# segments-ai/latent-diffusion-segmentation

Measured on AMD Instinct MI355X. Metric: denoising-steps/sec, higher is better.
Workload: dtype bf16; 1 GPU; 512x512 COCO-shaped latents (64x64x4), batch 8 per GPU, DDIM, self-conditioned 12-ch UNet without cross-attention (BASELINE configs[1]); batch_per_gpu=8, global_batch=8, latent=64, parallelism=dp1, ranks=1, backend=none, visible_devices=1

## Files before the change

include/ldmseg_hip_ops.h:

```cpp
#ifndef LDMSEG_HIP_OPS_H_
#define LDMSEG_HIP_OPS_H_
#include <stdint.h>
#ifdef __cplusplus
extern "C" {
#endif

int ldmseg_op_conv2d(const float* x, const float* x2, const float* w, const float* bias, int B, int Ci, int Ci2, int H,
                     int W, int Co, int k, int stride, int up, int dtype, float* out, void* stream);
int ldmseg_op_linear(const float* x, const float* w, const float* bias, const float* resid, const float* rowbias,
                     int rows_per_image, int M, int K, int N, int geglu, int silu, int splits, int dtype, float* out,
                     void* stream);
int ldmseg_op_chained_ff_out(const float* g, const float* h, const float* x, const float* w2, const float* b2, const float* wp,
                             const float* bp, int M, int C, int rows_per_image, int dtype, float* out, void* stream);
int ldmseg_op_groupnorm(const float* x, const float* x2, const float* gamma, const float* beta, int B, int C, int C2,
                        int HW, float eps, int silu, int dtype, float* out, void* stream);
int ldmseg_op_layernorm(const float* x, const float* gamma, const float* beta, int M, int C, float eps, int silu,
                        int dtype, float* out, void* stream);
int ldmseg_op_attention(const float* qkv, int B, int N, int C, int heads, int dtype, float* out, void* stream);
int ldmseg_op_attention_causal(const float* qkv, int B, int N, int C, int heads, int dtype, float* out, void* stream);
int ldmseg_op_attention_cross(const float* q, const float* kv, int B, int N, int S, int C, int heads, int dtype, float* out,
                              void* stream);
int ldmseg_op_attention_fp8(const float* qkv, int B, int N, int C, int heads, float* out, int time_iters, float* us_per_launch,
                            void* stream);
int ldmseg_op_convt2(const float* x, const float* w, const float* bias, int B, int Ci, int H, int W, int Co, int dtype,
// ... 41 lines not shown
                             const float* w2, const float* b2, const float* wp, const float* bp, int M, int C, float eps, int dtype,
                             int mode, float* out, int time_iters, float* us_per_call, void* stream);
int ldmseg_op_conv_out_tail(const float* x, const float* w, const float* bias, int B, int H, int W, float* eps_out, int ddim, int last,
                            const float* coef4, int pred_type, int clip, float clip_range, float* latents, float* cond,
                            const float* rgb, const uint8_t* known, const float* z0, const float* noise, float sa, float sb,
                            float* xin_out, void* stream);
int ldmseg_bench_igemm(const float* x, const float* x2, const float* w, const float* bias, const float* resid,
                       const float* rowbias, int B, int Ci, int Ci2, int H, int W, int Co, int k, int stride, int up, int geglu,
                       int silu, int splits, int dtype, int iters, float* us_per_launch, void* stream);
int ldmseg_bench_groupnorm(const float* gamma, const float* beta, int B, int C, int C2, int HW, int silu, int dtype, int iters,
                           float* us_per_launch, void* stream);
int ldmseg_bench_attention(const float* qkv, int B, int N, int C, int heads, int dtype, int iters, float* us_per_launch,
                           void* stream);
int ldmseg_igemm_last_kernel(char* buf, int n);
int ldmseg_op_igemm_plan(const int* desc, int dtype, int cus, char* buf, int n);
int ldmseg_op_groupnorm_plan(int B, int C, int C2, int HW, int groups, int dtype, int cus, int region_ok, char* buf, int n);
int ldmseg_op_conv_groupnorm_plan(int B, int Co, int HW, int dtype, char* buf, int n);
int ldmseg_op_attention_plan(int kind, int B, int N, int S, int C, int heads, int dtype, char* buf, int n);
int ldmseg_igemm_log(int enable);
int ldmseg_igemm_log_read(char* buf, int n);

int ldmseg_op_fastdiv(const int* n, int count, int d, int* q, void* stream);

#ifdef __cplusplus
}
#endif
#endif
```

latent-diffusion-segmentation_amd/csrc/engine.hip:

```cpp
#include <hip/hip_runtime.h>

#include <algorithm>
#include <array>
#include <cmath>
#include <cstdio>
#include <cstring>
#include <string>
#include <unordered_map>
#include <vector>

#include "../../include/ldmseg_hip.h"
#include "attn_plan.h"
#include "kernels.h"

using namespace ldmseg;

namespace {

thread_local std::string g_err;
int g_plan_epoch = 0;
int g_gnfold_mode = 1;
int g_ffp_mode = 1;
int fail(int code, const std::string& msg) {
  g_err = msg;
// ... 2423 lines not shown
  if (key == 8) { groupnorm_set_variant(value); ++g_plan_epoch; return 0; }
  if (key == 9) { igemm_set_cm_mode(value); ++g_plan_epoch; return 0; }
  if (key == 10) { groupnorm_set_coop(value, groupnorm_knob(11)); return 0; }
  if (key == 11) { groupnorm_set_coop(groupnorm_knob(10), value); return 0; }
  if (key == 12) { mlp_fused_set_mode(value); ++g_plan_epoch; return 0; }
  if (key == 13) { mlp_fused_set_dbg(value); return 0; }
  if (key == 14) { step_tail_set_mode(value); ++g_plan_epoch; return 0; }
  if (key == 16) { proj_qkv_set_mode(value); ++g_plan_epoch; return 0; }
  if (key == 15) { attention_mx_set_mode(value); ++g_plan_epoch; return 0; }
  if (key == 23) { igemm_set_cf_mode(value); ++g_plan_epoch; return 0; }
  if (key == 24) { igemm_set_table_override(value); ++g_plan_epoch; return 0; }
  if (key == 19) { igemm_set_xt_mode(value); ++g_plan_epoch; return 0; }
  if (key == 20) { g_ffp_mode = value ? 1 : 0; ++g_plan_epoch; return 0; }
  if (key == 22) { g_gnfold_mode = value < 0 ? 0 : value; ++g_plan_epoch; return 0; }
  if (key == 21) { igemm_set_up4_mode(value); ++g_plan_epoch; return 0; }
  if (key == 6 || key == 7) { ops_bench_knob(key, value); return 0; }
  static unsigned long long ts_ptr = 0;
  if (key == 3) { ts_ptr = (ts_ptr & 0xffffffff00000000ull) | (unsigned)value; igemm_set_tsbuf((void*)(uintptr_t)ts_ptr); return 0; }
  if (key == 4) { ts_ptr = (ts_ptr & 0xffffffffull) | ((unsigned long long)(unsigned)value << 32); igemm_set_tsbuf((void*)(uintptr_t)ts_ptr); return 0; }
  return fail(LDMSEG_E_ARG, "unknown debug key");
}

int ldmseg_debug_get(int key) {
  if (key == 1) return igemm_get_dbg();
  if (key == -1) return igemm_default_dbg();
  if (key == 8 || key == 11) return groupnorm_knob(key);
  if (key == 9) return igemm_get_cm_mode();
  if (key == 12) return mlp_fused_get_mode();
  if (key == 14) return step_tail_get_mode();
  if (key == 16) return proj_qkv_get_mode();
  if (key == 15) return attention_mx_get_mode();
  if (key == 23) return igemm_get_cf_mode();
  if (key == 19) return igemm_get_xt_mode();
  if (key == 20) return g_ffp_mode;
  if (key == 22) return g_gnfold_mode;
  if (key == 21) return igemm_get_up4_mode();
  if (key == 10) { const long long n = gn_coop_fallbacks(nullptr); return n > 0x7fffffffll ? 0x7fffffff : (int)n; }
  return 0;
}

int ldmseg_igemm_last_kernel(char* buf, int n) {
  if (!buf || n < 1) return LDMSEG_E_ARG;
  std::snprintf(buf, (size_t)n, "%s", igemm_dispatch_line(igemm_last_dispatch()).c_str());
  return 0;
}
int ldmseg_igemm_log(int enable) { igemm_log_enable(enable); return 0; }
int ldmseg_igemm_log_read(char* buf, int n) {
  if (!buf || n < 1) return LDMSEG_E_ARG;
  const std::string s = igemm_log_read();
  if ((int)s.size() + 1 > n) return LDMSEG_E_ARG;
  std::memcpy(buf, s.c_str(), s.size() + 1);
  return 0;
}

int ldmseg_profile_dump(const char* path) {
  g_err.clear();
  FILE* fp = std::fopen(path, "w");
  if (!fp) return fail(LDMSEG_E_ARG, "cannot open profile dump file");
// ... 17 lines not shown
```

latent-diffusion-segmentation_amd/csrc/igemm.hip:

```cpp
#include <cstdarg>
#include <cstdio>
#include <set>
#include <string>
#include <type_traits>

#include "common.h"
#include "igemm_plan.h"
#include "kernels.h"

namespace ldmseg {

namespace {

constexpr int kThreads = 256;
constexpr int kRowBytes = 128;

typedef __attribute__((address_space(1))) const void* gptr_t;
typedef __attribute__((address_space(3))) void* lptr_t;

__device__ __forceinline__ void glds16(const void* gsrc, unsigned lds_dst) {
  asm volatile(
      "s_mov_b32 m0, %1\n\t"
      "s_nop 0\n\t"
      "global_load_lds_dwordx4 %0, off"
// ... 1043 lines not shown
  static void* z[kMaxDev] = {};
  const int dev = cur_dev();
  if (!z[dev]) {
    if (hipMalloc(&z[dev], 64 << 10) != hipSuccess) return nullptr;
    (void)hipMemset(z[dev], 0, 64 << 10);
  }
  return z[dev];
}

}
std::string igemm_dispatch_name(const IgemmDispatch& d);
namespace {
int g_log_level = 0;
std::set<std::string> g_log;
IgemmDispatch g_last{};
int g_dbg = 0;
void* g_tsbuf = nullptr;
IgemmKnobs g_knobs;

IgemmLaunchDesc describe(const IgemmParams& p) {
  return {p.M, p.N, p.C0, p.C1, p.C2, p.C3, p.taps, p.stride, p.up, p.up4, p.cm, p.epi, p.rowstats ? 1 : 0, p.x3, p.splits, p.no_finish, p.cf_ctr ? 1 : 0};
}

template <typename T>
int launch_finish(const IgemmParams& p, hipStream_t s) {
  const int nq = p.n_valid >> 2;
  const int gx = (nq + 63) / 64;
  int gy = (p.M + 3) / 4;
  if (gy > 2048 / gx) gy = 2048 / gx > 0 ? 2048 / gx : 1;
  LDMSEG_LAUNCH(launch_name("splitk_finish<%s>", dtype_tag<T>()), splitk_finish_kernel<T>, dim3(gx, gy), dim3(256), 0, s, p);
// ... 72 lines not shown
#undef LDMSEG_IGEMM_LAUNCH_ROW
#undef LDMSEG_IGEMM_ON
  return -2;
}

}

int igemm_warm() { return zero_page() ? 0 : -3; }
const void* igemm_zero_page() { return zero_page(); }
void igemm_set_tsbuf(void* b) { g_tsbuf = b; }
void igemm_force_cfg(int cfg) { g_knobs.force_cfg = cfg; }
void igemm_set_dbg(int f) { g_dbg = f & 0xff; g_knobs.policy = (f >> 8) & 63; }
int igemm_get_dbg() { return (g_knobs.policy << 8) | g_dbg; }
int igemm_default_dbg() { return kDefaultPolicy << 8; }
IgemmDispatch igemm_last_dispatch() { return g_last; }
std::string igemm_dispatch_line(const IgemmDispatch& d) {
  return igemm_dispatch_name(d) + " splits=" + std::to_string(d.splits) + " grid=" + std::to_string(d.grid);
}
std::string igemm_dispatch_name(const IgemmDispatch& d) {
  char buf[112];
  std::snprintf(buf, sizeof buf, "igemm<%s,%d,%d,%d,%d,%d,%d,%d%s%s%s>%s", d.dtype == DT_BF16 ? "bf16" : "f32", d.bm, d.bn, d.wm, d.wn,
                d.nst, d.pipe, d.ldr, d.lnf ? ",ln" : "", d.cm ? ",cm" : (d.xt ? ",xt" : (d.up4 ? ",up4" : "")),
                d.x3 == 2 ? ",x3w" : (d.x3 ? ",x3" : ""), d.splits > 1 ? (d.cf ? "/splitk-cf" : "/splitk") : "");
  return buf;
}
void igemm_log_enable(int level) { g_log_level = level < 0 ? 0 : (level > 2 ? 2 : level); if (g_log_level) g_log.clear(); }
int igemm_log_level() { return g_log_level; }
void igemm_log_note(const char* name) { if (g_log_level) g_log.insert(name); }
std::string launch_name(const char* fmt, ...) {
  char buf[160];
// ... 157 lines not shown
  else hipLaunchKernelGGL(concat_rows_kernel<float>, dim3(g), dim3(256), 0, s, (const float*)a, K1, (const float*)b, K2, (float*)out, total);
  return hipGetLastError() == hipSuccess ? 0 : -3;
}

void igemm_set_cm_mode(int mode) { g_knobs.cm_mode = mode < -1 || mode > 1 ? -1 : mode; }
int igemm_get_cm_mode() { return g_knobs.cm_mode; }
bool igemm_conv_cm(int hw, int ctot, int n, int k, int stride, int up, int dtype) { return igemm_conv_cm_pure(g_knobs, hw, ctot, n, k, stride, up, dtype); }

int launch_igemm(const IgemmParams& p, int dtype, hipStream_t s) {
  if (p.up4 && (p.resid || p.rowbias || p.M != 4 * p.B * p.Ho * p.Wo || p.Hi != p.Ho || p.Wi != p.Wo)) return -2;
  if (p.cm && p.pad >= 0 && p.pad != 1) return -2;
  if (p.n_valid % 4 != 0 && p.epi != EPI_NCHW_F32) return -2;
  if (p.splits > 1 && p.partial == nullptr) return -2;
  if (p.rowstats && (!p.c1 || p.rowbias)) return -2;
  if ((p.C2 > 0 || p.C3 > 0) && !igemm_xt_ok(p, dtype)) return -2;
  IgemmDispatch d;
  if (const int r = igemm_choose(describe(p), dtype, g_knobs, num_cus(), &d)) return r;
  return launch_tile(d, p, s);
}

}
```

latent-diffusion-segmentation_amd/csrc/kernels.h:

```cpp
#pragma once
#include <hip/hip_runtime.h>
#include <stdint.h>

#include <string>
#include <vector>

#include "igemm_types.h"

namespace ldmseg {

struct FastDiv {
  unsigned mul = 0;
  int shift = 0;
  int d = 1;
};
inline FastDiv fastdiv_make(int d) {
  FastDiv f;
  f.d = d < 1 ? 1 : d;
  if (f.d == 1) return f;
  int s = 0;
  while ((1ll << s) < f.d) ++s;
  const unsigned long long num = 1ull << (31 + s);
  f.mul = (unsigned)((num + (unsigned long long)f.d - 1) / (unsigned long long)f.d);
  f.shift = s - 1;
// ... 82 lines not shown
std::string igemm_dispatch_line(const IgemmDispatch& d);
void igemm_log_enable(int level);
int igemm_log_level();
void igemm_log_note(const char* name);
std::string igemm_log_read();
std::string launch_name(const char* fmt, ...);
template <typename T>
constexpr const char* dtype_tag() { return sizeof(T) == 2 ? "bf16" : "f32"; }
#define LDMSEG_LAUNCH_AT(LEVEL, NAME, ...)                                                                  \
  do {                                                                                                      \
    if (::ldmseg::igemm_log_level() >= (LEVEL)) ::ldmseg::igemm_log_note(std::string(NAME).c_str());        \
    hipLaunchKernelGGL(__VA_ARGS__);                                                                        \
  } while (0)
#define LDMSEG_LAUNCH_GEMM(NAME, ...) LDMSEG_LAUNCH_AT(1, NAME, __VA_ARGS__)
#define LDMSEG_LAUNCH(NAME, ...) LDMSEG_LAUNCH_AT(2, NAME, __VA_ARGS__)
int igemm_pick_bn(int n_real, int epi);

struct GNParams {
  const void* src0 = nullptr; const void* src1 = nullptr;
  int C0 = 0, C1 = 0, B = 0, HW = 0, groups = 32;
  const float* gamma = nullptr; const float* beta = nullptr;
  float eps = 1e-5f; int silu = 0;
  void* out = nullptr;
  float* partial = nullptr;
  int nchunk = 0;
  int cpg = 0, vx = 0, ty = 0, per = 0;
  FastDiv fd_cpg, fd_vx, fd_aux;
  double inv_n = 0.0;
  void* sync_region = nullptr;
  unsigned long long* sync = nullptr;
// ... 185 lines not shown
```

latent-diffusion-segmentation_amd/csrc/ops_api.hip:

```cpp
#include <hip/hip_runtime.h>

#include <string>
#include <cstdio>
#include <cstdlib>
#include <cstring>
#include <vector>

#include "../../include/ldmseg_hip.h"
#include "common.h"
#include "attn_plan.h"
#include "gn_plan.h"
#include "kernels.h"

using namespace ldmseg;

static unsigned long long* op_cf_region() {
  static unsigned long long* r[64] = {};
  int dev = 0;
  if (hipGetDevice(&dev) != hipSuccess || dev < 0 || dev >= 64) return nullptr;
  if (!r[dev]) {
    void* q = nullptr;
    if (hipMalloc(&q, igemm_cf_bytes()) != hipSuccess) return nullptr;
    (void)hipMemset(q, 0, igemm_cf_bytes());
    r[dev] = (unsigned long long*)q;
// ... 456 lines not shown
    map.resize(Np, -1);
    const int* dmap = upload_map(t, map, s);
    if (launch_repack_rows(w, wp, dmap, Np, ct, dtype, s)) return -3;
    if (bias && launch_repack_rows(bias, bp, dmap, Np, 1, DT_F32, s)) return -3;
  } else if (!Ci2) {
    if (launch_repack_conv(w, wp, Co, Ci, k, k, Np, c0, dtype, s, cm ? a : 0)) return -3;
  } else {
    void* w_cat = t.get((size_t)Co * ct * k * k * sizeof(float));
    (void)hipMemsetAsync(w_cat, 0, (size_t)Co * ct * k * k * sizeof(float), s);
    (void)hipMemcpy2DAsync(w_cat, (size_t)ct * k * k * sizeof(float), w, (size_t)(Ci + Ci2) * k * k * sizeof(float),
                           (size_t)(Ci + Ci2) * k * k * sizeof(float), Co, hipMemcpyDeviceToDevice, s);
    if (launch_repack_conv((const float*)w_cat, wp, Co, ct, k, k, Np, ct, dtype, s, cm ? a : 0)) return -3;
  }
  const int Hl = up ? 2 * H : H, Wl = up ? 2 * W : W;
  const int Ho = (k == 3 && stride == 2) ? (Hl - 1) / 2 + 1 : Hl, Wo = (k == 3 && stride == 2) ? (Wl - 1) / 2 + 1 : Wl;
  void* rp = nullptr;
  if (resid) {
    rp = t.get((size_t)B * Ho * Wo * cout * es(dtype));
    if (launch_pack_nchw(resid, rp, B, cout, Ho * Wo, cout, 1.f, 0.f, dtype, s)) return -3;
  }
  void* op = t.get((size_t)B * Ho * Wo * cout * es(dtype));
  IgemmParams p;
  p.src0 = xp; p.C0 = c0; p.src1 = x2p; p.C1 = c1;
  p.B = B; p.Hi = H; p.Wi = W; p.Ho = Ho; p.Wo = Wo; p.taps = k * k; p.stride = stride; p.up = up; p.cm = cm ? 1 : 0;
  p.M = B * Ho * Wo; p.N = Np; p.n_valid = cout; p.W = wp; p.bias = bp;
  p.rowbias = rowbias; p.rb_stride = Co;
  p.resid = rp; p.ldr = cout; p.out = op; p.ldo = cout; p.epi = epi; p.silu = silu;
  p.x3 = x3;
  if (x3 == 2 && launch_split_planes(wp, (size_t)Np * k * k * ct, s)) return -3;
  if (up && k == 3 && stride == 1 && !Ci2 && !geglu && !resid && !rowbias && !silu && igemm_up4_ok(B, H, W, c0, Np, dtype) && Ci == c0) {
    void* w4 = t.get((size_t)16 * Np * c0 * es(dtype));
    if (launch_pack_up4(w, w4, Co, Ci, Np, c0, dtype, s)) return -3;
    p.W = w4; p.taps = 4; p.up = 0; p.up4 = 1; p.Ho = H; p.Wo = W; p.M = 4 * B * H * W; p.cm = 0;
  }
  p.cf_ctr = op_cf_region();
  int sp = splits > 0 ? splits : igemm_plan_splits(p, dtype);
// ... 64 lines not shown
  if (r) return r;
  if (iters > 0 && us_per_launch) *us_per_launch = time_launches(s, 0, iters, [&](int) { (void)launch_igemm(p, dtype, s); });
  if (!out) return 0;
  return unpack_nhwc(op, out, B, Co, HW, Co, dtype, s);
}

int ldmseg_op_igemm_plan(const int* desc, int dtype, int cus, char* buf, int n) {
  if (!desc || !buf || n < 1 || cus < 1 || dtype < 0 || dtype > 3) return -2;
  IgemmLaunchDesc q;
  static_assert(sizeof q == 17 * sizeof(int), "ldmseg_op_igemm_plan takes the fields of IgemmLaunchDesc in order");
  std::memcpy(&q, desc, sizeof q);
  if (dtype >= 2) { q.x3 = dtype - 1; dtype = DT_F32; }
  IgemmDispatch d;
  if (const int r = igemm_plan(q, dtype, cus, &d)) return r;
  std::snprintf(buf, (size_t)n, "%s", igemm_dispatch_line(d).c_str());
  return 0;
}

int ldmseg_op_fastdiv(const int* n, int count, int d, int* q, void* stream) {
  if (!n || !q || count < 0 || d < 1) return -2;
  const FastDiv f = fastdiv_make(d);
  hipLaunchKernelGGL(fastdiv_probe_kernel, dim3((count + 255) / 256), dim3(256), 0, (hipStream_t)stream, n, count, f, q);
  return hipGetLastError() == hipSuccess ? 0 : -3;
}
}
namespace ldmseg {
void ops_bench_knob(int key, int value) {
  if (key == 6) g_bench_rot = value;
  if (key == 7) g_bench_ln = value;
}
// ... 296 lines not shown
```

latent-diffusion-segmentation_amd/ldmseg_amd/_lib.py:

```python
import ctypes as C
import os

_HERE = os.path.dirname(os.path.abspath(__file__))
LIB_PATH = os.environ.get("LDMSEG_HIP_LIB") or os.path.join(_HERE, "libldmseg_hip.so")

F32, BF16, BF16X3 = 0, 1, 2
PRED = {"epsilon": 0, "sample": 1, "v_prediction": 2}


class UNetCfg(C.Structure):
    _fields_ = [("in_channels", C.c_int32), ("cross_attention", C.c_int32),
                ("compute_dtype", C.c_int32), ("device", C.c_int32)]


class VAECfg(C.Structure):
    _fields_ = [("in_channels", C.c_int32), ("int_channels", C.c_int32), ("out_channels", C.c_int32),
                ("latent_channels", C.c_int32), ("num_latents", C.c_int32), ("num_upscalers", C.c_int32),
                ("upscale_channels", C.c_int32), ("norm_num_groups", C.c_int32),
                ("block_out_channels", C.c_int32 * 4), ("compute_dtype", C.c_int32), ("device", C.c_int32)]


class VAEImageCfg(C.Structure):
    _fields_ = [("compute_dtype", C.c_int32), ("device", C.c_int32)]

# ... 98 lines not shown
    "ldmseg_op_conv_out_tail": (_i, [_vp, _vp, _vp, _i, _i, _i, _vp, _i, _i, C.POINTER(C.c_float), _i, _i, _f, _vp, _vp, _vp, _vp, _vp,
                                     _vp, _f, _f, _vp, _vp]),
    "ldmseg_op_transformer_ff": (_i, [_vp] * 10 + [_i, _i, _f, _i, _i, _vp, _i, C.POINTER(C.c_float), _vp]),
    "ldmseg_op_transformer_in": (_i, [_vp] * 8 + [_i, _i, _f, _i, _i, _vp, _vp, _i, C.POINTER(C.c_float), _vp]),
    "ldmseg_op_gn_transformer_in": (_i, [_vp] * 3 + [_f, _i, _i] + [_vp] * 7 + [_i, _i, _f, _i, _i, _vp, _vp, _i, C.POINTER(C.c_float), _vp]),
    "ldmseg_bench_igemm": (_i, [_vp, _vp, _vp, _vp, _vp, _vp, _i, _i, _i, _i, _i, _i, _i, _i, _i, _i, _i, _i, _i, _i,
                                C.POINTER(C.c_float), _vp]),
    "ldmseg_bench_attention": (_i, [_vp, _i, _i, _i, _i, _i, _i, C.POINTER(C.c_float), _vp]),
    "ldmseg_op_panoptic_from_decoder": (_i, [_vp, _i, _i, _i, _i, _i, _i, _i, _vp, _vp, _vp, _i, _i, _f, _i, _d, _i64, _vp, _vp, _vp,
                                             _vp, _vp, _vp, _vp]),
    "ldmseg_op_semseg_from_decoder": (_i, [_vp, _i, _i, _i, _i, _i, _i, _i, _f, _i64, _vp, _i64, _i, _vp, _vp, _vp, _vp]),
    "ldmseg_op_conv_groupnorm": (_i, [_vp, _vp, _vp, _vp, _vp, _vp, _i, _i, _i, _i, _i, _f, _i, _i, _i, _vp, _vp]),
    "ldmseg_bench_groupnorm": (_i, [_vp, _vp, _i, _i, _i, _i, _i, _i, _i, C.POINTER(C.c_float), _vp]),
    "ldmseg_igemm_last_kernel": (_i, [C.c_char_p, _i]),
    "ldmseg_op_igemm_plan": (_i, [C.POINTER(_i), _i, _i, C.c_char_p, _i]),
    "ldmseg_op_groupnorm_plan": (_i, [_i, _i, _i, _i, _i, _i, _i, _i, C.c_char_p, _i]),
    "ldmseg_op_conv_groupnorm_plan": (_i, [_i, _i, _i, _i, C.c_char_p, _i]),
    "ldmseg_op_attention_plan": (_i, [_i, _i, _i, _i, _i, _i, _i, C.c_char_p, _i]),
    "ldmseg_op_fastdiv": (_i, [_vp, _i, _i, _vp, _vp]),
    "ldmseg_igemm_log": (_i, [_i]),
    "ldmseg_igemm_log_read": (_i, [C.c_char_p, _i]),
}

_lib = None


def lib():
    global _lib
    if _lib is None:
        if not os.path.exists(LIB_PATH):
# ... 73 lines not shown
```

latent-diffusion-segmentation_amd/ldmseg_amd/build.py:

```python
import hashlib
import os
import subprocess
import sys
from concurrent.futures import ThreadPoolExecutor

HERE = os.path.dirname(os.path.abspath(__file__))
CSRC = os.path.normpath(os.path.join(HERE, "..", "csrc"))
INCLUDE = os.path.normpath(os.path.join(HERE, "..", "..", "include"))
LIB_PATH = os.path.join(HERE, "libldmseg_hip.so")
SOURCES = ["igemm.hip", "tfuse.hip", "tproj.hip", "tail.hip", "norm.hip", "attention.hip", "attention3.hip", "attention4.hip", "attention_fp8.hip", "attention_mx.hip", "attention_cross.hip", "clip_vision.hip", "clip_text.hip", "guided.hip", "misc.hip", "postproc.hip", "pq_meter.hip", "sched.hip", "engine.hip", "ops_api.hip"]
EXTRA_FLAGS = {
    "sched.hip": ["-ffp-contract=off"],
    "tail.hip": ["-ffp-contract=off"],
    "guided.hip": ["-ffp-contract=off"],
    "attention.hip": ["-mllvm", "-amdgpu-mfma-vgpr-form"],
    "attention3.hip": ["-mllvm", "-amdgpu-mfma-vgpr-form", "-fno-honor-nans"],
    "attention4.hip": ["-mllvm", "-amdgpu-mfma-vgpr-form", "-fno-honor-nans"],
    "attention_fp8.hip": ["-mllvm", "-amdgpu-mfma-vgpr-form", "-fno-honor-nans"],
    "attention_mx.hip": ["-mllvm", "-amdgpu-mfma-vgpr-form", "-fno-honor-nans"],
}
FLAGS = ["--offload-arch=gfx950", "-O3", "-std=c++17", "-fPIC", "-Wno-unused-result"]


def _hipcc():
    for cand in (os.environ.get("HIPCC"), "/opt/rocm/bin/hipcc", "hipcc"):
# ... 9 lines not shown
            h.update(b"\0" + os.path.basename(d).encode() + b"\0" + f.read())
    return h.hexdigest()


def _current(target, stamp, digest):
    if not (os.path.exists(target) and os.path.exists(stamp)):
        return False
    with open(stamp) as f:
        return f.read().strip() == digest


def build_library(force=False, verbose=False):
    hipcc = _hipcc()
    objdir = os.path.join(CSRC, "build")
    os.makedirs(objdir, exist_ok=True)
    headers = [os.path.join(CSRC, h) for h in ("common.h", "kernels.h", "igemm_types.h", "igemm_plan.h", "gn_plan.h", "attn_plan.h", "attn_dev.h", "igemm_tuned.inc", "sched_math.h")]
    headers += [os.path.join(INCLUDE, h) for h in ("ldmseg_hip.h", "ldmseg_hip_ops.h")]
    jobs = []
    objs = []
    for src in SOURCES:
        s = os.path.join(CSRC, src)
        o = os.path.join(objdir, src.replace(".hip", ".o"))
        objs.append(o)
        cmd = [hipcc] + FLAGS + EXTRA_FLAGS.get(src, []) + ["-c", s, "-o", o]
        dig = _digest(cmd, [s] + headers)
        if force or not _current(o, o + ".sha", dig):
            jobs.append((cmd, o + ".sha", dig))

    def run(cmd):
        if verbose:
            print(" ".join(cmd), file=sys.stderr)
# ... 31 lines not shown
```

Measured before the change: 1045 image-steps/s.

## Add dedicated DMA-ring bf16 1x1 GEMM kernel with per-shape tuned tiles

Adds a specialized GEMM kernel for plain 1x1/linear bf16 projections (store epilogue, optional residual). It uses global_load_lds direct-to-LDS transfers into a multi-stage ring, optional dedicated loader waves, and MFMA/ds_read interleaving, and picks its tile height from a per-shape tuned table. It is tried before the generic implicit-GEMM path and falls back when the shape or alignment is not supported. It also lets the residual reuse the output buffer when the two alias, saving one packing buffer. The cost is a second GEMM code path with inline asm and strict preconditions.

```diff
diff --git a/include/ldmseg_hip_ops.h b/include/ldmseg_hip_ops.h
--- a/include/ldmseg_hip_ops.h
+++ b/include/ldmseg_hip_ops.h
@@ -79,6 +79,7 @@
                            void* stream);
 int ldmseg_igemm_last_kernel(char* buf, int n);
 int ldmseg_op_igemm_plan(const int* desc, int dtype, int cus, char* buf, int n);
+int ldmseg_op_gemm1_plan(const int* desc, int dtype, int rowbias, int resid, int silu, int cus, char* buf, int n);
 int ldmseg_op_groupnorm_plan(int B, int C, int C2, int HW, int groups, int dtype, int cus, int region_ok, char* buf, int n);
 int ldmseg_op_conv_groupnorm_plan(int B, int Co, int HW, int dtype, char* buf, int n);
 int ldmseg_op_attention_plan(int kind, int B, int N, int S, int C, int heads, int dtype, char* buf, int n);
diff --git a/latent-diffusion-segmentation_amd/csrc/engine.hip b/latent-diffusion-segmentation_amd/csrc/engine.hip
--- a/latent-diffusion-segmentation_amd/csrc/engine.hip
+++ b/latent-diffusion-segmentation_amd/csrc/engine.hip
@@ -2461,6 +2461,7 @@
   if (key == 20) { g_ffp_mode = value ? 1 : 0; ++g_plan_epoch; return 0; }
   if (key == 22) { g_gnfold_mode = value < 0 ? 0 : value; ++g_plan_epoch; return 0; }
   if (key == 21) { igemm_set_up4_mode(value); ++g_plan_epoch; return 0; }
+  if (key == 25) { gemm1_set_mode(value); ++g_plan_epoch; return 0; }
   if (key == 6 || key == 7) { ops_bench_knob(key, value); return 0; }
   static unsigned long long ts_ptr = 0;
   if (key == 3) { ts_ptr = (ts_ptr & 0xffffffff00000000ull) | (unsigned)value; igemm_set_tsbuf((void*)(uintptr_t)ts_ptr); return 0; }
@@ -2482,13 +2483,14 @@
   if (key == 20) return g_ffp_mode;
   if (key == 22) return g_gnfold_mode;
   if (key == 21) return igemm_get_up4_mode();
+  if (key == 25) return gemm1_get_mode();
   if (key == 10) { const long long n = gn_coop_fallbacks(nullptr); return n > 0x7fffffffll ? 0x7fffffff : (int)n; }
   return 0;
 }
 
 int ldmseg_igemm_last_kernel(char* buf, int n) {
   if (!buf || n < 1) return LDMSEG_E_ARG;
-  std::snprintf(buf, (size_t)n, "%s", igemm_dispatch_line(igemm_last_dispatch()).c_str());
+  std::snprintf(buf, (size_t)n, "%s", igemm_last_line().c_str());
   return 0;
 }
 int ldmseg_igemm_log(int enable) { igemm_log_enable(enable); return 0; }
diff --git a/latent-diffusion-segmentation_amd/csrc/gemm1.hip b/latent-diffusion-segmentation_amd/csrc/gemm1.hip
--- /dev/null
+++ b/latent-diffusion-segmentation_amd/csrc/gemm1.hip
@@ -0,0 +1,332 @@
+#include <cstdio>
+#include <string>
+#include <type_traits>
+
+#include "common.h"
+#include "gemm1_plan.h"
+#include "kernels.h"
+
+namespace ldmseg {
+
+namespace {
+
+constexpr int kRowBytes = kGemm1RowBytes;
+
+struct Gemm1Params {
+  const void* X;
+  const void* W;
+  const float* bias;
+  const void* resid;
+  const void* zeros;
+  void* out;
+  int K, ldr, ldo, nk, nt;
+  FastDiv fd_nt;
+};
+
+__device__ __forceinline__ void dma16(unsigned voff, const void* sbase, unsigned lds_dst) {
+  asm volatile(
+      "s_mov_b32 m0, %2\n\t"
+      "s_nop 3\n\t"
+      "global_load_lds_dwordx4 %0, %1"
+      :
+      : "v"(voff), "s"(sbase), "s"(lds_dst)
+      : "memory");
+}
+template <int N>
+__device__ __forceinline__ void wait_vm() {
+  asm volatile("s_waitcnt vmcnt(%0)" ::"i"(N) : "memory");
+}
+template <int PER, int MAXN>
+__device__ __forceinline__ void wait_batches(int n) {
+  if constexpr (MAXN == 0) {
+    wait_vm<0>();
+  } else {
+    if (n >= MAXN) wait_vm<MAXN * PER>();
+    else wait_batches<PER, MAXN - 1>(n);
+  }
+}
+__device__ __forceinline__ void ring_barrier() { asm volatile("s_waitcnt lgkmcnt(0)\n\ts_barrier" ::: "memory"); }
+
+template <int BM, int BN, int WAVES_M, int WAVES_N, int LDR>
+__global__ __launch_bounds__((WAVES_M * WAVES_N + LDR) * 64, (WAVES_M * WAVES_N + LDR + 3) / 4) void gemm1_kernel(const Gemm1Params p) {
+  constexpr int NW = WAVES_M * WAVES_N;
+  static_assert(NW == 4 || NW == 8, "4 or 8 compute waves per workgroup");
+  constexpr int NLW = LDR ? LDR : NW;
+  constexpr int NST = gemm1_ring(BM);
+  constexpr int WTM = BM / WAVES_M, WTN = BN / WAVES_N;
+  constexpr int MF = WTM / 16, NF = WTN / 16;
+  constexpr int kStageBytes = (BM + BN) * kRowBytes;
+  static_assert(NST >= 2 && NST * kStageBytes <= kGemm1LdsBytes, "ring / LDS");
+
+  extern __shared__ __attribute__((aligned(16))) unsigned char smem[];
+
+  const int tid = threadIdx.x;
+  const int lane = tid & 63;
+  const int wave_id = __builtin_amdgcn_readfirstlane(tid >> 6);
+  const bool is_ldr = LDR ? wave_id >= NW : true;
+  const int wave = LDR ? (wave_id < NW ? wave_id : wave_id - NW) : wave_id;
+  const int wm = wave / WAVES_N, wn = wave % WAVES_N;
+
+  int tile;
+  {
+    const int G = gridDim.x, bid = blockIdx.x;
+    const int q = G >> 3, r = G & 7, xcd = bid & 7, idx = bid >> 3;
+    tile = (xcd < r ? xcd * (q + 1) : r * (q + 1) + (xcd - r) * q) + idx;
+  }
+  const int mt = fd_div(tile, p.fd_nt);
+  const int m0 = mt * BM, n0 = (tile - mt * p.nt) * BN;
+
+  constexpr int XG = BM / 8 / NLW;
+  constexpr int WGN = BN / 8;
+  constexpr int WG = (WGN + NLW - 1) / NLW;
+  constexpr int WREM = WGN % NLW;
+  static_assert(BM % (8 * NLW) == 0 && BN % 8 == 0, "tile rows / loading waves");
+  const int ld_r = lane >> 3;
+  const int ld_j = (lane & 7) ^ ld_r;
+  const bool w_last = (WREM == 0) || (wave < WREM);
+  const unsigned lds_wave = __builtin_amdgcn_readfirstlane(
+      (unsigned)(uintptr_t)((__attribute__((address_space(3))) unsigned char*)smem) + (unsigned)wave * 1024u);
+  const unsigned row_bytes = (unsigned)p.K * 2u;
+  unsigned xoff[XG], woff[WG];
+#pragma unroll
+  for (int i = 0; i < XG; ++i) xoff[i] = (unsigned)((i * NLW + wave) * 8 + ld_r) * row_bytes + (unsigned)ld_j * 16u;
+#pragma unroll
+  for (int i = 0; i < WG; ++i) woff[i] = (unsigned)((i * NLW + wave) * 8 + ld_r) * row_bytes + (unsigned)ld_j * 16u;
+  const unsigned char* xtile = (const unsigned char*)p.X + (size_t)m0 * row_bytes;
+  const unsigned char* wtile = (const unsigned char*)p.W + (size_t)n0 * row_bytes;
+
+  auto sgpr_ptr = [&](const unsigned char* q) __attribute__((always_inline)) -> const unsigned char* {
+    const unsigned long long u = (unsigned long long)(uintptr_t)q;
+    const unsigned lo = __builtin_amdgcn_readfirstlane((unsigned)u), hi = __builtin_amdgcn_readfirstlane((unsigned)(u >> 32));
+    return (const unsigned char*)(uintptr_t)(((unsigned long long)hi << 32) | lo);
+  };
+  auto issue = [&](int kt, int stage) __attribute__((always_inline)) {
+    const unsigned dst = __builtin_amdgcn_readfirstlane(lds_wave + (unsigned)stage * (unsigned)kStageBytes);
+    const unsigned char* xt = sgpr_ptr(xtile + (size_t)kt * kRowBytes);
+    const unsigned char* wt = sgpr_ptr(wtile + (size_t)kt * kRowBytes);
+#pragma unroll
+    for (int i = 0; i < XG; ++i) dma16(xoff[i], xt, dst + i * (NLW * 1024));
+    const unsigned wdst = dst + BM * kRowBytes;
+#pragma unroll
+    for (int i = 0; i < WG; ++i)
+      if (i + 1 < WG || w_last) dma16(woff[i], wt, wdst + i * (NLW * 1024));
+  };
+  auto wait_tiles = [&](int n) __attribute__((always_inline)) {
+    if constexpr (WREM == 0) {
+      wait_batches<XG + WG, NST - 1>(n);
+    } else {
+      if (w_last) wait_batches<XG + WG, NST - 1>(n);
+      else wait_batches<XG + WG - 1, NST - 1>(n);
+    }
+  };
+
+  const int nk = p.nk;
+  const int npro = nk < NST ? nk : NST;
+  if constexpr (LDR > 0) {
+    if (wave_id >= NW) {
+#pragma unroll
+      for (int j = 0; j < NST; ++j)
+        if (j < npro) issue(j, j);
+      wait_tiles(npro - 1);
+      ring_barrier();
+      int st = 0;
+      for (int kt = 0; kt < nk; ++kt) {
+        const int behind = nk - 2 - kt;
+        wait_tiles(behind < 0 ? 0 : (behind < NST - 2 ? behind : NST - 2));
+        ring_barrier();
+        if (kt + NST < nk) issue(kt + NST, st);
+        st = (st + 1 == NST) ? 0 : st + 1;
+      }
+      return;
+    }
+  }
+
+  constexpr int E = 8;
+  constexpr int SROW = WTN * 4 + 16;
+  constexpr int CPR = WTN / E;
+  constexpr int NCH = 16 * CPR;
+  constexpr int NI = (NCH + 63) / 64;
+  static_assert(WTN % E == 0 && NW * 16 * SROW <= NST * kStageBytes, "row-major epilogue staging");
+  const int lq = lane & 15, lg = lane >> 4;
+  const int nw0 = n0 + wn * WTN;
+  const int m_wave = m0 + wm * WTM;
+  f32x4 bv[NF];
+#pragma unroll
+  for (int a = 0; a < NF; ++a) bv[a] = *(const f32x4*)(p.bias + nw0 + lg * 4 + a * 16);
+  const bool has_res = p.resid != nullptr;
+  auto load_res = [&](int b, uint4 (&r)[NI]) __attribute__((always_inline)) {
+#pragma unroll
+    for (int i = 0; i < NI; ++i) {
+      const int c = lane + i * 64;
+      const int row = c / CPR, cc = c - row * CPR;
+      const bf16_t* rp = (const bf16_t*)p.resid + (size_t)(m_wave + b * 16 + row) * p.ldr + nw0 + cc * E;
+      if (c < NCH) r[i] = *(const uint4*)(has_res ? rp : (const bf16_t*)p.zeros);
+    }
+  };
+  uint4 rcur[NI], rnext[NI];
+  load_res(0, rcur);
+
+  if (is_ldr) {
+#pragma unroll
+    for (int j = 0; j < NST; ++j)
+      if (j < npro) issue(j, j);
+    wait_tiles(npro - 1);
+  }
+  ring_barrier();
+
+  f32x4 acc[NF][MF];
+#pragma unroll
+  for (int a = 0; a < NF; ++a)
+#pragma unroll
+    for (int b = 0; b < MF; ++b) acc[a][b] = f32x4{0.f, 0.f, 0.f, 0.f};
+
+  const int fr_row = (lane & 15) * kRowBytes;
+  const int fr_c0 = ((lane >> 4) ^ (lane & 7)) * 16;
+  const int fr_c1 = (((lane >> 4) + 4) ^ (lane & 7)) * 16;
+
+  uint4 wfA[NF], xfA[MF], wfB[NF], xfB[MF];
+#define GEMM1_READ(WF, XF, STAGE, CO)                                                                  \
+  {                                                                                                    \
+    const unsigned char* xs_ = smem + (STAGE) * kStageBytes + (wm * WTM) * kRowBytes + fr_row + (CO);  \
+    const unsigned char* ws_ = smem + (STAGE) * kStageBytes + (BM + wn * WTN) * kRowBytes + fr_row + (CO); \
+    WF[0] = *(const uint4*)(ws_);                                                                      \
+    _Pragma("unroll") for (int b = 0; b < MF; ++b) XF[b] = *(const uint4*)(xs_ + b * 16 * kRowBytes); \
+    _Pragma("unroll") for (int a = 1; a < NF; ++a) WF[a] = *(const uint4*)(ws_ + a * 16 * kRowBytes); \
+  }
+#define GEMM1_MMA(WF, XF)                                                                              \
+  _Pragma("unroll") for (int a = 0; a < NF; ++a)                                                       \
+    _Pragma("unroll") for (int b = 0; b < MF; ++b) mma_kgroup<bf16_t>(WF[a], XF[b], acc[a][b]);
+  constexpr int NMMA = NF * MF;
+  constexpr int MPR = NMMA / (NF + MF);
+#define GEMM1_INTERLEAVE                                                                               \
+  static_for_n<NF + MF>([&](auto) __attribute__((always_inline)) {                                     \
+    __builtin_amdgcn_sched_group_barrier(0x100, 1, 0);                                                 \
+    __builtin_amdgcn_sched_group_barrier(0x008, MPR, 0);                                               \
+  });                                                                                                  \
+  __builtin_amdgcn_sched_group_barrier(0x008, NMMA - MPR * (NF + MF), 0);                              \
+  __builtin_amdgcn_sched_barrier(0);
+
+  int cur = 0;
+  GEMM1_READ(wfA, xfA, cur, fr_c0)
+  for (int kt = 0; kt < nk; ++kt) {
+    GEMM1_READ(wfB, xfB, cur, fr_c1)
+    GEMM1_MMA(wfA, xfA)
+    GEMM1_INTERLEAVE
+    if (is_ldr) {
+      const int behind = nk - 2 - kt;
+      wait_tiles(behind < 0 ? 0 : (behind < NST - 2 ? behind : NST - 2));
+    }
+    ring_barrier();
+    if (is_ldr && kt + NST < nk) issue(kt + NST, cur);
+    cur = (cur + 1 == NST) ? 0 : cur + 1;
+    GEMM1_READ(wfA, xfA, cur, fr_c0)
+    GEMM1_MMA(wfB, xfB)
+    GEMM1_INTERLEAVE
+  }
+#undef GEMM1_READ
+#undef GEMM1_MMA
+#undef GEMM1_INTERLEAVE
+
+  unsigned char* stg = smem + wave * (16 * SROW);
+  auto row_block = [&](int b, auto bidx) __attribute__((always_inline)) {
+    constexpr int BI = decltype(bidx)::value;
+    const int mb = m_wave + b * 16;
+#pragma unroll
+    for (int a = 0; a < NF; ++a) *(f32x4*)(stg + lq * SROW + (a * 16 + lg * 4) * 4) = acc[a][BI] + bv[a];
+    if (b + 1 < MF) load_res(b + 1, rnext);
+    asm volatile("s_waitcnt lgkmcnt(0)" ::: "memory");
+#pragma unroll
+    for (int i = 0; i < NI; ++i) {
+      const int c = lane + i * 64;
+      if (c < NCH) {
+        const int row = c / CPR, cc = c - row * CPR;
+        float v[E];
+        const unsigned char* sp = stg + row * SROW + cc * E * 4;
+#pragma unroll
+        for (int q = 0; q < E / 4; ++q) {
+          const f32x4 t = *(const f32x4*)(sp + q * 16);
+          v[q * 4 + 0] = t[0]; v[q * 4 + 1] = t[1]; v[q * 4 + 2] = t[2]; v[q * 4 + 3] = t[3];
+        }
+        if (has_res) {
+          float r[E];
+          Chunk<bf16_t>::unpack(rcur[i], r);
+#pragma unroll
+          for (int e = 0; e < E; ++e) v[e] += r[e];
+        }
+        *(uint4*)((bf16_t*)p.out + (size_t)(mb + row) * p.ldo + nw0 + cc * E) = Chunk<bf16_t>::pack(v);
+      }
+    }
+    asm volatile("s_waitcnt lgkmcnt(0)" ::: "memory");
+#pragma unroll
+    for (int i = 0; i < NI; ++i) rcur[i] = rnext[i];
+  };
+  if constexpr (MF <= 2) {
+#pragma unroll 1
+    for (int b = 0; b < MF; ++b) {
+      row_block(b, std::integral_constant<int, 0>{});
+#pragma unroll
+      for (int a = 0; a < NF; ++a)
+#pragma unroll
+        for (int j = 0; j + 1 < MF; ++j) acc[a][j] = acc[a][j + 1];
+    }
+  } else {
+    static_for_n<MF>([&](auto bi) __attribute__((always_inline)) { row_block(decltype(bi)::value, bi); });
+  }
+}
+
+Gemm1Knobs g_knobs;
+
+std::string plan_name(const Gemm1Plan& pl) {
+  char buf[96];
+  std::snprintf(buf, sizeof buf, "gemm1<bf16,%d,%d,%d,%d,%d,%d>", pl.bm, pl.bn, pl.wm, pl.wn, pl.nst, pl.ldr);
+  return buf;
+}
+std::string plan_line(const Gemm1Plan& pl) { return plan_name(pl) + " splits=1 grid=" + std::to_string(pl.grid); }
+
+Gemm1Desc describe(const IgemmLaunchDesc& q, int dtype, int rowbias, int resid, int silu) { return Gemm1Desc{q, dtype, rowbias, resid, silu}; }
+
+template <int BM, int WM, int WN, int LDR>
+int run(const Gemm1Plan& pl, const Gemm1Params& gp, hipStream_t s) {
+  auto kern = gemm1_kernel<BM, kGemm1Bn, WM, WN, LDR>;
+  static bool attr_set[64] = {};
+  raise_lds_limit_once((const void*)kern, (size_t)gemm1_ring(BM) * gemm1_stage_bytes(BM), attr_set);
+  LDMSEG_LAUNCH_GEMM(plan_name(pl), kern, dim3(pl.grid), dim3((WM * WN + LDR) * 64), (size_t)pl.lds_bytes, s, gp);
+  return hipGetLastError() == hipSuccess ? 0 : -3;
+}
+
+}
+
+void gemm1_set_mode(int mode) { g_knobs.mode = mode < 0 ? 0 : mode; }
+int gemm1_get_mode() { return g_knobs.mode; }
+
+int gemm1_plan(const IgemmLaunchDesc& q, int dtype, int rowbias, int resid, int silu, int cus, std::string* line) {
+  Gemm1Plan pl;
+  if (!gemm1_choose(describe(q, dtype, rowbias, resid, silu), g_knobs, cus, &pl)) return 1;
+  if (line) *line = plan_line(pl) + " lds=" + std::to_string(pl.lds_bytes);
+  return 0;
+}
+
+int launch_gemm1(const IgemmParams& p, int dtype, hipStream_t s, std::string* line) {
+  if ((g_knobs.mode & 0xff) == 0) return 1;
+  const IgemmLaunchDesc q{p.M, p.N, p.C0, p.C1, p.C2, p.C3, p.taps, p.stride, p.up, p.up4, p.cm, p.epi, p.rowstats ? 1 : 0, p.x3, p.splits, p.no_finish, p.cf_ctr ? 1 : 0};
+  Gemm1Plan pl;
+  if (!gemm1_choose(describe(q, dtype, p.rowbias ? 1 : 0, p.resid ? 1 : 0, p.silu), g_knobs, num_cus(), &pl)) return 1;
+  auto al16 = [](const void* a) { return ((uintptr_t)a & 15) == 0; };
+  if (p.n_valid != p.N || p.ldo < p.N || p.ldo % 8 != 0 || (p.resid && (p.ldr < p.N || p.ldr % 8 != 0))) return 1;
+  if (!p.src0 || !p.W || !p.out || !al16(p.src0) || !al16(p.W) || !al16(p.out) || !al16(p.resid) || !al16(p.bias)) return 1;
+  Gemm1Params gp;
+  gp.X = p.src0; gp.W = p.W; gp.resid = p.resid; gp.out = p.out;
+  gp.zeros = igemm_zero_page();
+  if (!gp.zeros) return -3;
+  gp.bias = p.bias ? p.bias : (const float*)gp.zeros;
+  gp.K = p.C0; gp.ldr = p.ldr; gp.ldo = p.ldo; gp.nk = p.C0 / 64; gp.nt = p.N / pl.bn;
+  gp.fd_nt = fastdiv_make(gp.nt);
+  if (line) *line = plan_line(pl);
+#define LDMSEG_GEMM1_LAUNCH_ROW(BM, WM, WN, LDR) \
+  if (pl.bm == BM) return run<BM, WM, WN, LDR>(pl, gp, s);
+  LDMSEG_GEMM1_FORMS(LDMSEG_GEMM1_LAUNCH_ROW)
+#undef LDMSEG_GEMM1_LAUNCH_ROW
+  return -2;
+}
+
+}
diff --git a/latent-diffusion-segmentation_amd/csrc/gemm1_plan.h b/latent-diffusion-segmentation_amd/csrc/gemm1_plan.h
--- /dev/null
+++ b/latent-diffusion-segmentation_amd/csrc/gemm1_plan.h
@@ -0,0 +1,81 @@
+#pragma once
+#include "igemm_types.h"
+
+namespace ldmseg {
+
+constexpr int kGemm1DefaultMode = 1;
+struct Gemm1Knobs { int mode = kGemm1DefaultMode; };
+
+struct Gemm1Desc { IgemmLaunchDesc q; int dtype, rowbias, resid, silu; };
+
+struct Gemm1Plan { int bm, bn, wm, wn, nst, ldr, grid, lds_bytes; };
+
+constexpr int kGemm1Bn = 160;
+constexpr int kGemm1RowBytes = 128;
+constexpr int kGemm1LdsBytes = 160 << 10;
+constexpr int kGemm1MaxK = 1280;
+
+#define LDMSEG_GEMM1_FORMS(X) \
+  X(64, 2, 2, 4)              \
+  X(128, 4, 2, 0)             \
+  X(256, 4, 2, 0)
+struct Gemm1Form { int bm, wm, wn, ldr; };
+#define LDMSEG_GEMM1_FORM_ROW(BM, WM, WN, LDR) {BM, WM, WN, LDR},
+constexpr Gemm1Form kGemm1Forms[] = {LDMSEG_GEMM1_FORMS(LDMSEG_GEMM1_FORM_ROW)};
+#undef LDMSEG_GEMM1_FORM_ROW
+constexpr int kGemm1NumForms = (int)(sizeof(kGemm1Forms) / sizeof(kGemm1Forms[0]));
+
+constexpr int gemm1_stage_bytes(int bm) { return (bm + kGemm1Bn) * kGemm1RowBytes; }
+constexpr int gemm1_ring(int bm) { return kGemm1LdsBytes / gemm1_stage_bytes(bm); }
+constexpr int gemm1_epi_bytes(int wm, int wn) { return wm * wn * 16 * ((kGemm1Bn / wn) * 4 + 16); }
+static_assert(gemm1_ring(64) == 5 && gemm1_ring(128) == 4 && gemm1_ring(256) == 3, "ring depths of the three forms");
+
+struct Gemm1Tuned { int M, N, K, resid, bm; };
+constexpr Gemm1Tuned kGemm1Tuned[] = {
+#include "gemm1_tuned.inc"
+    {0, 0, 0, 0, 0}};
+
+inline bool gemm1_capable(const Gemm1Desc& d) {
+  const IgemmLaunchDesc& q = d.q;
+  if (d.dtype != DT_BF16 || q.x3) return false;
+  if (q.taps != 1 || q.stride != 1 || q.up || q.up4 || q.cm) return false;
+  if (q.C1 || q.C2 || q.C3 || q.splits > 1) return false;
+  if (q.epi != EPI_STORE || q.lnf || d.rowbias || d.silu) return false;
+  if (q.M <= 0 || q.N <= 0 || q.M % 64 != 0 || q.N % kGemm1Bn != 0) return false;
+  return q.C0 % 64 == 0 && q.C0 >= 64 && q.C0 <= kGemm1MaxK;
+}
+
+inline int gemm1_form_of(int bm) {
+  for (int f = 0; f < kGemm1NumForms; ++f)
+    if (kGemm1Forms[f].bm == bm) return f;
+  return -1;
+}
+
+inline bool gemm1_choose(const Gemm1Desc& d, const Gemm1Knobs& k, int cus, Gemm1Plan* plan) {
+  const int mode = k.mode & 0xff;
+  if (mode != 1 && mode != 2) return false;
+  if (!gemm1_capable(d)) return false;
+  const int M = d.q.M, N = d.q.N, K = d.q.C0;
+  int bm = 0;
+  if (mode == 1) {
+    for (const Gemm1Tuned* e = kGemm1Tuned; e->M > 0; ++e)
+      if (e->M == M && e->N == N && e->K == K && e->resid == (d.resid ? 1 : 0)) bm = e->bm;
+  } else if (k.mode >> 8) {
+    bm = k.mode >> 8;
+  } else {
+    bm = 64;
+    for (int f = kGemm1NumForms - 1; f >= 0; --f)
+      if (M % kGemm1Forms[f].bm == 0 && (long)(M / kGemm1Forms[f].bm) * (N / kGemm1Bn) >= cus) { bm = kGemm1Forms[f].bm; break; }
+  }
+  const int f = gemm1_form_of(bm);
+  if (f < 0 || M % bm != 0) return false;
+  const long grid = (long)(M / bm) * (N / kGemm1Bn);
+  if (grid > 0x7fffffffl) return false;
+  const Gemm1Form& t = kGemm1Forms[f];
+  const int nk = K / 64, ring = gemm1_ring(bm), used = nk + 1 < ring ? nk + 1 : ring;
+  const int ring_bytes = used * gemm1_stage_bytes(bm), epi = gemm1_epi_bytes(t.wm, t.wn);
+  *plan = Gemm1Plan{bm, kGemm1Bn, t.wm, t.wn, ring, t.ldr, (int)grid, ring_bytes > epi ? ring_bytes : epi};
+  return true;
+}
+
+}
diff --git a/latent-diffusion-segmentation_amd/csrc/gemm1_tuned.inc b/latent-diffusion-segmentation_amd/csrc/gemm1_tuned.inc
--- /dev/null
+++ b/latent-diffusion-segmentation_amd/csrc/gemm1_tuned.inc
@@ -0,0 +1,9 @@
+    {32768, 320, 320, 1, 256},
+    {8192, 640, 640, 1, 128},
+    {2048, 1280, 1280, 0, 64},
+    {2048, 1280, 1280, 1, 64},
+    {512, 1280, 1280, 0, 64},
+    {512, 1280, 1280, 1, 64},
+    {16384, 640, 640, 1, 256},
+    {1024, 1280, 1280, 0, 64},
+    {1024, 1280, 1280, 1, 64},
diff --git a/latent-diffusion-segmentation_amd/csrc/igemm.hip b/latent-diffusion-segmentation_amd/csrc/igemm.hip
--- a/latent-diffusion-segmentation_amd/csrc/igemm.hip
+++ b/latent-diffusion-segmentation_amd/csrc/igemm.hip
@@ -1081,6 +1081,7 @@
 int g_log_level = 0;
 std::set<std::string> g_log;
 IgemmDispatch g_last{};
+std::string g_last_gemm1;
 int g_dbg = 0;
 void* g_tsbuf = nullptr;
 IgemmKnobs g_knobs;
@@ -1183,6 +1184,7 @@
 int igemm_get_dbg() { return (g_knobs.policy << 8) | g_dbg; }
 int igemm_default_dbg() { return kDefaultPolicy << 8; }
 IgemmDispatch igemm_last_dispatch() { return g_last; }
+std::string igemm_last_line() { return g_last_gemm1.empty() ? igemm_dispatch_line(g_last) : g_last_gemm1; }
 std::string igemm_dispatch_line(const IgemmDispatch& d) {
   return igemm_dispatch_name(d) + " splits=" + std::to_string(d.splits) + " grid=" + std::to_string(d.grid);
 }
@@ -1370,6 +1372,8 @@
   if (p.splits > 1 && p.partial == nullptr) return -2;
   if (p.rowstats && (!p.c1 || p.rowbias)) return -2;
   if ((p.C2 > 0 || p.C3 > 0) && !igemm_xt_ok(p, dtype)) return -2;
+  g_last_gemm1.clear();
+  if (const int r = launch_gemm1(p, dtype, s, &g_last_gemm1); r != 1) return r;
   IgemmDispatch d;
   if (const int r = igemm_choose(describe(p), dtype, g_knobs, num_cus(), &d)) return r;
   return launch_tile(d, p, s);
diff --git a/latent-diffusion-segmentation_amd/csrc/kernels.h b/latent-diffusion-segmentation_amd/csrc/kernels.h
--- a/latent-diffusion-segmentation_amd/csrc/kernels.h
+++ b/latent-diffusion-segmentation_amd/csrc/kernels.h
@@ -120,6 +120,11 @@
   } while (0)
 #define LDMSEG_LAUNCH_GEMM(NAME, ...) LDMSEG_LAUNCH_AT(1, NAME, __VA_ARGS__)
 #define LDMSEG_LAUNCH(NAME, ...) LDMSEG_LAUNCH_AT(2, NAME, __VA_ARGS__)
+int launch_gemm1(const IgemmParams& p, int dtype, hipStream_t s, std::string* line);
+int gemm1_plan(const IgemmLaunchDesc& q, int dtype, int rowbias, int resid, int silu, int cus, std::string* line);
+void gemm1_set_mode(int mode);
+int gemm1_get_mode();
+std::string igemm_last_line();
 int igemm_pick_bn(int n_real, int epi);
 
 struct GNParams {
diff --git a/latent-diffusion-segmentation_amd/csrc/ops_api.hip b/latent-diffusion-segmentation_amd/csrc/ops_api.hip
--- a/latent-diffusion-segmentation_amd/csrc/ops_api.hip
+++ b/latent-diffusion-segmentation_amd/csrc/ops_api.hip
@@ -494,12 +494,12 @@
   }
   const int Hl = up ? 2 * H : H, Wl = up ? 2 * W : W;
   const int Ho = (k == 3 && stride == 2) ? (Hl - 1) / 2 + 1 : Hl, Wo = (k == 3 && stride == 2) ? (Wl - 1) / 2 + 1 : Wl;
+  void* op = t.get((size_t)B * Ho * Wo * cout * es(dtype));
   void* rp = nullptr;
   if (resid) {
-    rp = t.get((size_t)B * Ho * Wo * cout * es(dtype));
+    rp = (const void*)resid == (const void*)out && !time_iters ? op : t.get((size_t)B * Ho * Wo * cout * es(dtype));
     if (launch_pack_nchw(resid, rp, B, cout, Ho * Wo, cout, 1.f, 0.f, dtype, s)) return -3;
   }
-  void* op = t.get((size_t)B * Ho * Wo * cout * es(dtype));
   IgemmParams p;
   p.src0 = xp; p.C0 = c0; p.src1 = x2p; p.C1 = c1;
   p.B = B; p.Hi = H; p.Wi = W; p.Ho = Ho; p.Wo = Wo; p.taps = k * k; p.stride = stride; p.up = up; p.cm = cm ? 1 : 0;
@@ -594,6 +594,18 @@
   IgemmDispatch d;
   if (const int r = igemm_plan(q, dtype, cus, &d)) return r;
   std::snprintf(buf, (size_t)n, "%s", igemm_dispatch_line(d).c_str());
+  return 0;
+}
+
+int ldmseg_op_gemm1_plan(const int* desc, int dtype, int rowbias, int resid, int silu, int cus, char* buf, int n) {
+  if (!desc || !buf || n < 1 || cus < 1 || dtype < 0 || dtype > 3) return -2;
+  IgemmLaunchDesc q;
+  std::memcpy(&q, desc, sizeof q);
+  if (dtype >= 2) { q.x3 = dtype - 1; dtype = DT_F32; }
+  std::string line;
+  buf[0] = 0;
+  if (gemm1_plan(q, dtype, rowbias, resid, silu, cus, &line)) return 1;
+  std::snprintf(buf, (size_t)n, "%s", line.c_str());
   return 0;
 }
 
diff --git a/latent-diffusion-segmentation_amd/ldmseg_amd/_lib.py b/latent-diffusion-segmentation_amd/ldmseg_amd/_lib.py
--- a/latent-diffusion-segmentation_amd/ldmseg_amd/_lib.py
+++ b/latent-diffusion-segmentation_amd/ldmseg_amd/_lib.py
@@ -136,6 +136,7 @@
     "ldmseg_bench_groupnorm": (_i, [_vp, _vp, _i, _i, _i, _i, _i, _i, _i, C.POINTER(C.c_float), _vp]),
     "ldmseg_igemm_last_kernel": (_i, [C.c_char_p, _i]),
     "ldmseg_op_igemm_plan": (_i, [C.POINTER(_i), _i, _i, C.c_char_p, _i]),
+    "ldmseg_op_gemm1_plan": (_i, [C.POINTER(_i), _i, _i, _i, _i, _i, C.c_char_p, _i]),
     "ldmseg_op_groupnorm_plan": (_i, [_i, _i, _i, _i, _i, _i, _i, _i, C.c_char_p, _i]),
     "ldmseg_op_conv_groupnorm_plan": (_i, [_i, _i, _i, _i, C.c_char_p, _i]),
     "ldmseg_op_attention_plan": (_i, [_i, _i, _i, _i, _i, _i, _i, C.c_char_p, _i]),
diff --git a/latent-diffusion-segmentation_amd/ldmseg_amd/build.py b/latent-diffusion-segmentation_amd/ldmseg_amd/build.py
--- a/latent-diffusion-segmentation_amd/ldmseg_amd/build.py
+++ b/latent-diffusion-segmentation_amd/ldmseg_amd/build.py
@@ -8,7 +8,7 @@
 CSRC = os.path.normpath(os.path.join(HERE, "..", "csrc"))
 INCLUDE = os.path.normpath(os.path.join(HERE, "..", "..", "include"))
 LIB_PATH = os.path.join(HERE, "libldmseg_hip.so")
-SOURCES = ["igemm.hip", "tfuse.hip", "tproj.hip", "tail.hip", "norm.hip", "attention.hip", "attention3.hip", "attention4.hip", "attention_fp8.hip", "attention_mx.hip", "attention_cross.hip", "clip_vision.hip", "clip_text.hip", "guided.hip", "misc.hip", "postproc.hip", "pq_meter.hip", "sched.hip", "engine.hip", "ops_api.hip"]
+SOURCES = ["igemm.hip", "gemm1.hip", "tfuse.hip", "tproj.hip", "tail.hip", "norm.hip", "attention.hip", "attention3.hip", "attention4.hip", "attention_fp8.hip", "attention_mx.hip", "attention_cross.hip", "clip_vision.hip", "clip_text.hip", "guided.hip", "misc.hip", "postproc.hip", "pq_meter.hip", "sched.hip", "engine.hip", "ops_api.hip"]
 EXTRA_FLAGS = {
     "sched.hip": ["-ffp-contract=off"],
     "tail.hip": ["-ffp-contract=off"],
@@ -48,7 +48,7 @@
     hipcc = _hipcc()
     objdir = os.path.join(CSRC, "build")
     os.makedirs(objdir, exist_ok=True)
-    headers = [os.path.join(CSRC, h) for h in ("common.h", "kernels.h", "igemm_types.h", "igemm_plan.h", "gn_plan.h", "attn_plan.h", "attn_dev.h", "igemm_tuned.inc", "sched_math.h")]
+    headers = [os.path.join(CSRC, h) for h in ("common.h", "kernels.h", "igemm_types.h", "igemm_plan.h", "gemm1_plan.h", "gemm1_tuned.inc", "gn_plan.h", "attn_plan.h", "attn_dev.h", "igemm_tuned.inc", "sched_math.h")]
     headers += [os.path.join(INCLUDE, h) for h in ("ldmseg_hip.h", "ldmseg_hip_ops.h")]
     jobs = []
     objs = []
```

Measured after the change: 1051 image-steps/s (median of 6 runs). No clear change (+0.6%).
